# MCG-NJU/SparseBEV

Hardware: AMD Instinct MI355X
Metric: decoder samples/sec (6-cam T=8 900q r50_704x256, 6 layers, features resident in HBM) (higher is better)
Workload: dtype f32 (the two mixing GEMMs: f16x3 = fp32-class (default): fp32 operands as scaled fp16 hi + lo images, 3 products (hl, lh, hh), f32 accumulate on the 16-bit matrix core (csrc/gemm_bf16s.hip); max and rms error vs fp64 below the exact f32 MFMA kernels (tests/test_gpu_bf16s.py); mixing generator + out-; 1 GPU; c2: r50_704x256, 900 queries, T=8, bs=1 per GPU, 6 decoder layers, random-init weights, NCHW (reference layout, relayout inside the step: on demand -- only the feature units the sample points read) feature input; global_batch=1, parallelism=sample-sharded x1, launches_per_layer=6, query_order=False, shuffled_queries=False, relayout=on-demand

## Files before the change

### sparsebev_amd/csrc/gemm_bf16s.hip

```cpp
#include <atomic>
#include <cstdlib>
#include <type_traits>
#include "sbev_common.hpp"

#ifdef SBEV_EXP_NOSTORE
#define SBEV_EXP_STORE_COND && a.M < 0
#else
#define SBEV_EXP_STORE_COND
#endif
#ifdef SBEV_EXP_NOMFMA
#define SBEV_MFMA(A, B, C) ([&]() { asm volatile("" ::"v"(A), "v"(B)); return C; }())
#else
#define SBEV_MFMA(A, B, C) mfma16<PR::F16>(A, B, C)
#endif

#ifdef SBEV_EXP_TRACE
__device__ unsigned long long g_sbev_trace[2][512][8];
#define SBEV_TRACE(G_, SLOT_)                                                                               \
    if (blockIdx.x == 0 && (wave & 3) == 0 && lane == 0 && (G_) < 512) g_sbev_trace[wave >> 2][G_][SLOT_] = __builtin_readcyclecounter();
extern "C" int sbev_debug_trace_read(unsigned long long* out) {
    return (int)hipMemcpyFromSymbol(out, HIP_SYMBOL(g_sbev_trace), sizeof(g_sbev_trace));
}
#else
#define SBEV_TRACE(G_, SLOT_)
// ... 286 lines not shown
    typedef Fmt<MODE> PR;
    constexpr int NIMG = PR::NIMG;
    constexpr bool F16 = PR::F16;
    extern __shared__ __attribute__((aligned(16))) unsigned char lds[];
    constexpr Gen3Lds L{NIMG, RF};
    constexpr int AF = 2 * RF;
    constexpr int STAGE = L.stage();
    constexpr int NST = L.depth();
    constexpr bool EPI_LDS = L.patches();
    constexpr int EPI_LD = Gen3Lds::EPI_LD;
    constexpr int SLICES = L.slices_at();
    constexpr bool ISSUE_IN_COMPUTE = false;
    constexpr bool SPLIT_ACC = RF == 2;
    constexpr int NBLK = AF + 8;
    constexpr int NLMAX = (NBLK + 7) / 8;
    const int tid = threadIdx.x, lane = tid & 63;
    const int wave = __builtin_amdgcn_readfirstlane(tid >> 6);
    const int wr = wave >> 2, wc = wave & 3;
    SBEV_WGTIME(0, 0)
    const int M = a.M, nk = a.K / 16;
    const int lw = (int)xcd_contiguous(blockIdx.x, gridDim.x);
    const int rt = lw % a.ntm, ct0 = lw / a.ntm, cstep = (int)gridDim.x / a.ntm, nct = a.N / G_COLS;
    const int my_tiles = ct0 < nct ? (nct - ct0 + cstep - 1) / cstep : 0;
    const int G = my_tiles * nk;
    if (G == 0) return;
    const int f0 = a.rows.first(rt), nf = a.rows.count(rt);
    const int m0 = f0 * 32;
    int nfa = nf - RF * wr;
    nfa = nfa < 0 ? 0 : (nfa > RF ? RF : nfa);
    const int nlb = (NBLK - wave + 7) / 8;
    const int nl = nlb * NIMG;

    const unsigned voff = (unsigned)lane * 16u;
    const unsigned char* gbase[NLMAX];
    unsigned ldst[NLMAX];
    long long gstep[NLMAX];
    const int nfrag = (M + 31) / 32;
    const long long blkbytes = (long long)nk * NIMG * 1024;
#pragma unroll
    for (int j = 0; j < NLMAX; ++j) {
        const int q = wave + 8 * j;
        ldst[j] = (unsigned)(q * NIMG * 1024);
        if (q < AF) {
            int fb = f0 + q;
            fb = fb < nfrag ? fb : nfrag - 1;
            gbase[j] = reinterpret_cast<const unsigned char*>(a.Xs) + fb * blkbytes;
            gstep[j] = -(long long)nk * NIMG * 1024;
        } else {
            gbase[j] = reinterpret_cast<const unsigned char*>(a.Ws) + (long long)(ct0 * 8 + (q - AF)) * blkbytes;
            gstep[j] = (long long)(cstep * 8) * blkbytes - (long long)nk * NIMG * 1024;
        }
    }
    int lk = 0, lg = 0;
    auto issue_next = [&]() {
        if (lg >= G) return;
        const unsigned sb = (unsigned)((lg % NST) * STAGE);
#pragma unroll
        for (int j = 0; j < NLMAX; ++j) {
#ifndef SBEV_EXP_NOGLDS
            if (j < nlb) lds_dma<NIMG>(gbase[j], voff, sb + ldst[j]);
#endif
            gbase[j] += NIMG * 1024;
        }
        ++lg;
        if (++lk == nk) {
            lk = 0;
#pragma unroll
            for (int j = 0; j < NLMAX; ++j) gbase[j] += gstep[j];
        }
    };
    const int l31 = lane & 31, lh = lane >> 5;
    const unsigned aoff = (unsigned)(wr * RF) * (NIMG * 1024u) + voff;
    const unsigned boff = (unsigned)(AF + wc * 2) * (NIMG * 1024u) + voff;

    auto run = [&](auto nfa_c) {
        constexpr int NFA = decltype(nfa_c)::value;
        constexpr int NFR = NFA > 0 ? NFA : 1;
        bf16x8 xf[NFR][NIMG], wf[2][NIMG];
        constexpr int NFS = SPLIT_ACC ? NFR : 1;
        f32x16 acc[NFR][2], accs[NFS][2];
        auto init_acc = [&](int ti) {
#pragma unroll
            for (int fb = 0; fb < 2; ++fb) {
                const float bv = F16 ? 0.f : reinterpret_cast<const float*>(lds + SLICES)[ti * G_COLS + (wc * 2 + fb) * 32 + l31];
#pragma unroll
                for (int fa = 0; fa < NFR; ++fa)
#pragma unroll
                    for (int e = 0; e < 16; ++e) {
                        acc[fa][fb][e] = bv;
                        if constexpr (SPLIT_ACC) accs[fa][fb][e] = 0.f;
                    }
            }
        };
        auto store_tile = [&](int n0, int tix) {
            if constexpr (NFA > 0) {
                if constexpr (F16) {
                    const float* bs = reinterpret_cast<const float*>(lds + SLICES) + tix * G_COLS + wc * 64 + l31;
                    const float* cs = bs + my_tiles * G_COLS;
                    const float b0 = bs[0], b1 = bs[32], c0 = cs[0], c1 = cs[32];
#pragma unroll
                    for (int fa = 0; fa < NFA; ++fa)
#pragma unroll
                        for (int e = 0; e < 16; ++e) {
                            acc[fa][0][e] = fmaf(acc[fa][0][e], c0, b0);
                            acc[fa][1][e] = fmaf(acc[fa][1][e], c1, b1);
                        }
                }
                if (a.relu) {
#pragma unroll
                    for (int fa = 0; fa < NFA; ++fa)
#pragma unroll
                        for (int fb = 0; fb < 2; ++fb)
#pragma unroll
                            for (int e = 0; e < 16; ++e) acc[fa][fb][e] = fmaxf(acc[fa][fb][e], 0.f);
                }
                if constexpr (EPI_LDS) {
                    float* patch = reinterpret_cast<float*>(lds + NST * STAGE) + wave * (32 * EPI_LD);
                    const int pr = lane >> 3, pc = (lane & 7) * 4;
#pragma unroll
                    for (int fa = 0; fa < NFA; ++fa) {
                        const int r0 = m0 + (wr * RF + fa) * 32;
#pragma unroll
                        for (int fb = 0; fb < 2; ++fb) {
#pragma unroll
                            for (int e = 0; e < 16; ++e) patch[((e & 3) + 8 * (e >> 2) + 4 * lh) * EPI_LD + l31] = acc[fa][fb][e];
                            __builtin_amdgcn_wave_barrier();
                            f32x4 v[4];
#pragma unroll
                            for (int i = 0; i < 4; ++i) v[i] = *reinterpret_cast<const f32x4*>(patch + (pr + 8 * i) * EPI_LD + pc);
                            __builtin_amdgcn_wave_barrier();
                            float* y = a.Y + (long long)(r0 + pr) * a.ldy + n0 + wc * 64 + fb * 32 + pc;
#pragma unroll
                            for (int i = 0; i < 4; ++i)
                                if (r0 + pr + 8 * i < M SBEV_EXP_STORE_COND) *reinterpret_cast<f32x4*>(y + (long long)(8 * i) * a.ldy) = v[i];
                        }
                    }
                    return;
                }
#pragma unroll
                for (int fa = 0; fa < NFA; ++fa) {
                    const int r0 = m0 + (wr * RF + fa) * 32;
                    float* y = a.Y + (long long)(r0 + 4 * lh) * a.ldy + n0 + wc * 64 + l31;
                    if (r0 + 32 <= M SBEV_EXP_STORE_COND) {
#pragma unroll
                        for (int e = 0; e < 16; ++e) {
                            y[0] = acc[fa][0][e];
                            y[32] = acc[fa][1][e];
                            y += (e & 3) == 3 ? 5 * a.ldy : a.ldy;
                            asm volatile("" : "+v"(y));
                        }
                    } else {
#pragma unroll
                        for (int e = 0; e < 16; ++e) {
                            if (r0 + 4 * lh + (e & 3) + 8 * (e >> 2) < M SBEV_EXP_STORE_COND) {
                                y[0] = acc[fa][0][e];
                                y[32] = acc[fa][1][e];
                            }
                            y += (e & 3) == 3 ? 5 * a.ldy : a.ldy;
                            asm volatile("" : "+v"(y));
                        }
                    }
                }
            }
        };
        int cn0 = ct0 * G_COLS, ck = 0, ti = 0;
        bool pending = false;
        for (int i = tid; i < my_tiles * G_COLS; i += 512) {
            const int t = i / G_COLS, c = i - t * G_COLS;
            reinterpret_cast<float*>(lds + SLICES)[i] = a.bias ? a.bias[(ct0 + t * cstep) * G_COLS + c] : 0.f;
            if constexpr (F16)
                reinterpret_cast<float*>(lds + SLICES)[my_tiles * G_COLS + i] = a.colscale[(ct0 + t * cstep) * G_COLS + c] * a.xscale[1];
        }
        __syncthreads();
        init_acc(0);
#pragma unroll
        for (int i = 0; i < NST - 1; ++i) issue_next();
        wait_vmcnt_imm<0>();
        __syncthreads();
        if (wr == 1) phase_barrier();
        for (int g = 0; g < G; ++g) {
            SBEV_TRACE(g, 0)
            if constexpr (NFA > 0) {
                const unsigned char* st = lds + (g % NST) * STAGE;
#pragma unroll
                for (int img = 0; img < NIMG; ++img) {
                    wf[0][img] = *reinterpret_cast<const bf16x8*>(st + boff + img * 1024);
                    wf[1][img] = *reinterpret_cast<const bf16x8*>(st + boff + (NIMG + img) * 1024);
#pragma unroll
                    for (int fa = 0; fa < NFA; ++fa) xf[fa][img] = *reinterpret_cast<const bf16x8*>(st + aoff + (fa * NIMG + img) * 1024);
                }
            }
            SBEV_TRACE(g, 1)
            if constexpr (!ISSUE_IN_COMPUTE) issue_next();
            SBEV_TRACE(g, 2)
            {
                const int hi = lg - 1, need = g + 1 < G ? g + 1 : g;
                wait_vmcnt_n(hi > need ? (hi - need) * nl : 0);
            }
            if (pending) {
                store_tile(cn0, ti);
                cn0 += cstep * G_COLS;
                ++ti;
                init_acc(ti < my_tiles ? ti : 0);
                pending = false;
            }
            SBEV_TRACE(g, 3)
            phase_barrier();
            SBEV_TRACE(g, 4)
            if constexpr (ISSUE_IN_COMPUTE) issue_next();
            if constexpr (NFA > 0) {
#pragma unroll
                for (int p = 0; p < PR::N - 1; ++p)
#pragma unroll
                    for (int fa = 0; fa < NFA; ++fa)
#pragma unroll
                        for (int fb = 0; fb < 2; ++fb) {
                            if constexpr (SPLIT_ACC) accs[fa][fb] = SBEV_MFMA(xf[fa][PR::ia(p)], wf[fb][PR::ib(p)], accs[fa][fb]);
                            else acc[fa][fb] = SBEV_MFMA(xf[fa][PR::ia(p)], wf[fb][PR::ib(p)], acc[fa][fb]);
                        }
#pragma unroll
                for (int fa = 0; fa < NFA; ++fa)
#pragma unroll
                    for (int fb = 0; fb < 2; ++fb)
                        acc[fa][fb] = SBEV_MFMA(xf[fa][0], wf[fb][0], acc[fa][fb]);
            }
            if (++ck == nk) {
                ck = 0;
                pending = true;
                if constexpr (NFA > 0 && SPLIT_ACC) {
#pragma unroll
                    for (int fa = 0; fa < NFA; ++fa)
#pragma unroll
                        for (int fb = 0; fb < 2; ++fb) acc[fa][fb] += accs[fa][fb];
                }
            }
            SBEV_TRACE(g, 5)
            phase_barrier();
            SBEV_TRACE(g, 6)
        }
        if (wr == 0) phase_barrier();
        if (pending) store_tile(cn0, ti);
        SBEV_WGTIME(0, 1)
    };
    if (nfa == RF) run(std::integral_constant<int, RF>{});
    else if (nfa == RF - 1) run(std::integral_constant<int, RF - 1>{});
    else if (nfa == 0) run(std::integral_constant<int, 0>{});
    else if constexpr (RF == 4) {
        if (nfa == 2) run(std::integral_constant<int, 2>{});
        else run(std::integral_constant<int, 1>{});
    }
}

struct GenWsArgs {
    const unsigned short* Xs;
    const unsigned short* Ws;
    const float* bias;
    float* Y;
    int M, N;
    long long ldy;
    int relu;
    int nrs; RowSplit rows;
    int ntask;
    const float* colscale;
    const float* xscale;
    int lazy_on, lazy_esize;
    LazyArgs lazy;
    const uint32_t* skip_hdr;
};

#ifndef SBEV_WS_NCH
#define SBEV_WS_NCH 2
#endif
constexpr int WS_KS = 16;
constexpr int WS_FRAG = WS_KS * 2 * 1024;
constexpr int WS_SLOTS = 4;
constexpr int WS_LDS = WS_SLOTS * WS_FRAG;
static_assert(WS_LDS <= Gen3Lds::BUDGET, "the X ring fits the CU's LDS");

__device__ __forceinline__ void lds_barrier() {
    __builtin_amdgcn_sched_barrier(0);
    asm volatile("s_waitcnt lgkmcnt(0)\n\ts_barrier" ::: "memory");
    __builtin_amdgcn_sched_barrier(0);
}

template <int MODE, bool RELU>
__global__ __launch_bounds__(512) void gemm_f16s_gen_ws_kernel(const GenWsArgs a) {
    typedef Fmt<MODE> PR;
    static_assert(PR::NIMG == 2, "two-image modes only: the stationary weights are 128 registers");
    constexpr bool F16 = PR::F16;
    extern __shared__ __attribute__((aligned(16))) unsigned char lds[];
    if (a.skip_hdr && sbev::prefix_clean(a.skip_hdr)) return;
    const int lane = threadIdx.x & 63;
    const int wave = __builtin_amdgcn_readfirstlane((int)threadIdx.x >> 6);
    const int l31 = lane & 31, lh = lane >> 5;
    const unsigned voff = (unsigned)lane * 16u;
    const unsigned long long yb = (unsigned long long)a.Y;
    __amdgpu_buffer_rsrc_t yrs = __builtin_amdgcn_make_buffer_rsrc(
        reinterpret_cast<void*>(((unsigned long long)(unsigned)__builtin_amdgcn_readfirstlane((int)(unsigned)(yb >> 32)) << 32) |
                                (unsigned)__builtin_amdgcn_readfirstlane((int)(unsigned)yb)),
        0, (int)(unsigned)((long long)a.M * a.ldy * 4), 0x00020000);
    const unsigned ldyb = (unsigned)(a.ldy * 4);
    [[maybe_unused]] const int tid = (int)threadIdx.x;
    SBEV_WGTIME(1, 0)
    if (a.lazy_on) {
        float* wt = reinterpret_cast<float*>(lds);
        unsigned* list = reinterpret_cast<unsigned*>(lds + 8 * (LZ_TS * WLD * 4));
        unsigned* n_list = list + 4 * 512;
        if (a.lazy_esize == 4) lazy_scan_share<float>(a.lazy, blockIdx.x, gridDim.x, 512, wt, list, n_list);
        else lazy_scan_share<unsigned short>(a.lazy, blockIdx.x, gridDim.x, 512, wt, list, n_list);
        asm volatile("s_waitcnt vmcnt(0)" ::: "memory");
        __syncthreads();
    }

    {
        for (int task = (int)xcd_contiguous(blockIdx.x, gridDim.x); task < a.ntask; task += (int)gridDim.x) {
            const int ct = task / a.nrs, rs = task - ct * a.nrs;
            const int f0 = a.rows.first(rs), nf = a.rows.count(rs);
            if (nf <= 0) continue;
            const int n = ct * G_COLS + wave * 32 + l31;
            const float bv = a.bias ? a.bias[n] : 0.f;
            const float cv = F16 ? a.colscale[n] * a.xscale[1] : 1.f;
            const unsigned ycol = (unsigned)(4 * lh) * ldyb + (unsigned)n * 4u;
            const unsigned char* xg = reinterpret_cast<const unsigned char*>(a.Xs) + (long long)f0 * WS_FRAG + wave * 4096;
            auto issue = [&](int i) {
#ifndef SBEV_EXP_NOGLDS
                lds_dma<4>(xg + (long long)i * WS_FRAG, voff, (unsigned)((i % WS_SLOTS) * WS_FRAG + wave * 4096));
#endif
            };
            issue(0);
            if (nf > 1) issue(1);
            if (nf > 2) issue(2);
            __builtin_amdgcn_sched_barrier(0);
            bf16x8 wf[WS_KS][2];
            {
                const unsigned short* wb = a.Ws + ((long long)(ct * 8 + wave) * (WS_KS * 2) * 64 + lane) * 8;
#pragma unroll
                for (int ks = 0; ks < WS_KS; ++ks)
#pragma unroll
                    for (int img = 0; img < 2; ++img) wf[ks][img] = *reinterpret_cast<const bf16x8*>(wb + (ks * 2 + img) * 512);
            }
            __builtin_amdgcn_sched_barrier(0);
            wait_vmcnt_imm<32>();
            lds_barrier();
            f32x16 prev;
#pragma unroll
            for (int e = 0; e < 16; ++e) prev[e] = 0.f;
            for (int i = 0; i < nf; ++i) {
                SBEV_TRACE(i, 0)
                const unsigned char* st = lds + (i % WS_SLOTS) * WS_FRAG + voff;
                const unsigned yprev = i > 0 ? ycol + (unsigned)((f0 + i - 1) * 32) * ldyb : (ycol | 0x80000000u);
                constexpr int NCH = SBEV_WS_NCH;
                f32x16 accs[NCH];
#pragma unroll
                for (int c = 0; c < NCH; ++c)
#pragma unroll
                    for (int e = 0; e < 16; ++e) accs[c][e] = (F16 || c > 0) ? 0.f : bv;
                constexpr int NBLK = WS_KS / NCH;
                static_assert(WS_KS % NCH == 0 && NBLK % 2 == 0 && 16 % (NBLK / 2) == 0, "NCH divides the k-steps into an even number of blocks");
                constexpr int SPB = 16 / (NBLK / 2);
                bf16x8 xr[2][NCH][2];
#pragma unroll
                for (int c = 0; c < NCH; ++c) {
                    xr[0][c][0] = *reinterpret_cast<const bf16x8*>(st + (c * 2) * 1024);
                    xr[0][c][1] = *reinterpret_cast<const bf16x8*>(st + (c * 2 + 1) * 1024);
                }
#pragma unroll
                for (int blk = 0; blk < NBLK; ++blk) {
#ifndef SBEV_EXP_NOREAD
                    if (blk + 1 < NBLK) {
#pragma unroll
                        for (int c = 0; c < NCH; ++c) {
                            xr[(blk + 1) & 1][c][0] = *reinterpret_cast<const bf16x8*>(st + (((blk + 1) * NCH + c) * 2) * 1024);
                            xr[(blk + 1) & 1][c][1] = *reinterpret_cast<const bf16x8*>(st + (((blk + 1) * NCH + c) * 2 + 1) * 1024);
                        }
                    }
#endif
                    if (blk < NBLK / 2) {
#pragma unroll
                        for (int e = SPB * (blk % (NBLK / 2)); e < SPB * (blk % (NBLK / 2)) + SPB; ++e) {
                            const unsigned ro = (unsigned)((e & 3) + 8 * (e >> 2)) * ldyb;
#ifndef SBEV_EXP_NOSTORE
                            __builtin_amdgcn_raw_buffer_store_b32(__float_as_uint(prev[e]), yrs, (int)(yprev + ro), 0, 0);
#endif
                        }
                    }
#ifdef SBEV_EXP_NOREAD
                    const auto& xc = xr[0];
#else
                    const auto& xc = xr[blk & 1];
#endif
#pragma unroll
                    for (int p = 0; p < PR::N; ++p)
#pragma unroll
                        for (int c = 0; c < NCH; ++c) {
                            const int ks = blk * NCH + c;
                            if (p < PR::N - 1) accs[c] = SBEV_MFMA(xc[c][PR::ia(p)], wf[ks][PR::ib(p)], accs[c]);
                            else accs[c] = SBEV_MFMA(xc[c][0], wf[ks][0], accs[c]);
                        }
                    __builtin_amdgcn_sched_barrier(0);
                    if (blk == NBLK - 1) {
                        SBEV_TRACE(i, 1)
                        if (i + 2 < nf) wait_vmcnt_imm<4>();
                        else wait_vmcnt_imm<0>();
                        SBEV_TRACE(i, 2)
                        lds_barrier();
                        SBEV_TRACE(i, 3)
                        if (i + 3 < nf) issue(i + 3);
                        __builtin_amdgcn_sched_barrier(0);
                        SBEV_TRACE(i, 4)
                    }
                }
                f32x16 acc = accs[0];
#pragma unroll
                for (int c = 1; c < NCH; ++c) acc += accs[c];
#pragma unroll
                for (int e = 0; e < 16; ++e) {
                    const float v = F16 ? fmaf(acc[e], cv, bv) : acc[e];
                    prev[e] = RELU ? fmaxf(v, 0.f) : v;
                }
            }
            {
                const unsigned ylast = ycol + (unsigned)((f0 + nf - 1) * 32) * ldyb;
#pragma unroll
                for (int e = 0; e < 16; ++e)
                    __builtin_amdgcn_raw_buffer_store_b32(__float_as_uint(prev[e]), yrs, (int)(ylast + (unsigned)((e & 3) + 8 * (e >> 2)) * ldyb), 0, 0);
            }
        }
    }
    SBEV_WGTIME(1, 1)
}

struct OutArgs {
    const float* X;
    const unsigned short* Wp;
    float* P;
    int M, K;
    long long ldx;
    int nrt, S;
    float xup;
    const float* nscale;
    const float* xdev;
};

constexpr int O_IMG = 64 * 64;

template <int MODE>
__global__ __launch_bounds__(512) void gemm_bf16s_out3_kernel(const OutArgs a) {
    typedef Fmt<MODE> PR;
    constexpr int NIMG = PR::NIMG;
    extern __shared__ __attribute__((aligned(16))) unsigned char lds[];
    constexpr int HSTAGE = NIMG * O_IMG;
    constexpr int NST = 3;
    const int tid = threadIdx.x, lane = tid & 63;
    const int wave = __builtin_amdgcn_readfirstlane(tid >> 6);
    const int half = wave >> 2, wc = wave & 3;
    SBEV_WGTIME(2, 0)
    const unsigned logical = xcd_contiguous(blockIdx.x, gridDim.x);
    const int chunk = (int)(logical / (unsigned)a.nrt), rt = (int)(logical % (unsigned)a.nrt);
    const int M = a.M;
    const int m0 = rt * 64;
    const int nfa = (M - m0) > 32 ? 2 : 1;
    const int nslab = a.K / 32;
    const int c0 = (int)((long long)nslab * chunk / a.S), c1 = (int)((long long)nslab * (chunk + 1) / a.S);
    const int n_all = c1 - c0, n0h = (n_all + 1) / 2;
    const int sb = half == 0 ? c0 : c0 + n0h;
    const int nh = half == 0 ? n0h : n_all - n0h;

    const int th = tid & 255;
    const int srow = th >> 2, skq = th & 3;
    int grow = m0 + srow;
    grow = grow < M ? grow : M - 1;
    const float* xp = a.X + (long long)grow * a.ldx + skq * 8;
    const unsigned wofs = (unsigned)(srow * 64 + ((skq ^ ((srow >> 2) & 3)) * 16));
    unsigned char* hst = lds + half * (NST * HSTAGE);
    const int last_slab = nh > 0 ? sb + nh - 1 : c1 - 1;
    auto loadx = [&](int i, f32x4& v0, f32x4& v1) {
        int sl = sb + i;
        sl = sl < last_slab ? sl : last_slab;
#ifdef SBEV_EXP_HOTX
        sl = sl & 7;
#endif
        const float* p = xp + (long long)sl * 32;
        v0 = __builtin_nontemporal_load(reinterpret_cast<const f32x4*>(p));
        v1 = __builtin_nontemporal_load(reinterpret_cast<const f32x4*>(p + 4));
    };
    const float xup = a.xdev ? a.xdev[0] : a.xup;
    auto stagex = [&](int i, const f32x4 v0, const f32x4 v1) {
        u32x4 im[NIMG];
        split8m<MODE>(v0, v1, xup, im);
        unsigned char* st = hst + (i % NST) * HSTAGE + wofs;
#pragma unroll
        for (int img = 0; img < NIMG; ++img) *reinterpret_cast<u32x4*>(st + img * O_IMG) = im[img];
    };
    const int KS = a.K / 16;
    const unsigned short* wb0 = a.Wp + ((long long)(2 * wc) * KS * NIMG * 64 + lane) * 8;
    const unsigned short* wb1 = a.Wp + ((long long)(2 * wc + 1) * KS * NIMG * 64 + lane) * 8;
    auto loadw = [&](int i, int j, bf16x8 (&w)[2][NIMG]) {
        int sl = sb + i;
        sl = sl < last_slab ? sl : last_slab;
#ifdef SBEV_EXP_HOTW
        sl = sl & 7;
#endif
        const long long o = (long long)(2 * sl + j) * NIMG * 64 * 8;
#pragma unroll
        for (int img = 0; img < NIMG; ++img) {
            w[0][img] = *reinterpret_cast<const bf16x8*>(wb0 + o + img * 512);
            w[1][img] = *reinterpret_cast<const bf16x8*>(wb1 + o + img * 512);
        }
    };
    const int l31 = lane & 31, lh = lane >> 5;
    const unsigned swz = (unsigned)((lane >> 2) & 3);
    const unsigned fo0 = (unsigned)l31 * 64u + (((unsigned)lh) ^ swz) * 16u;
    const unsigned fo1 = (unsigned)l31 * 64u + ((2u + (unsigned)lh) ^ swz) * 16u;

    auto run = [&](auto nfa_c) {
        constexpr int NFA = decltype(nfa_c)::value;
        f32x16 acc[NFA][2];
#pragma unroll
        for (int fa = 0; fa < NFA; ++fa)
#pragma unroll
            for (int fb = 0; fb < 2; ++fb)
#pragma unroll
                for (int e = 0; e < 16; ++e) acc[fa][fb][e] = 0.f;
        f32x4 xa0, xa1, xb0, xb1;
        bf16x8 w[2][2][NIMG], xf[2][NFA][NIMG];
        loadx(0, xa0, xa1);
        loadx(1, xb0, xb1);
        loadw(0, 0, w[0]);
        loadw(0, 1, w[1]);
        stagex(0, xa0, xa1);
        loadx(2, xa0, xa1);
        stagex(1, xb0, xb1);
        loadx(3, xb0, xb1);
        __syncthreads();
        if (half == 1) phase_barrier();
#define SBEV_O3_SLAB(S_, X0, X1)                                                                            \
        {                                                                                                   \
                                                                                                 \
            {                                                                                               \
                SBEV_TRACE(S_, 0)                                                                           \
                const unsigned char* A = hst + ((S_) % NST) * HSTAGE;                                       \
                _Pragma("unroll") for (int img = 0; img < NIMG; ++img)                                      \
                    _Pragma("unroll") for (int fa = 0; fa < NFA; ++fa) {                                    \
                        xf[0][fa][img] = *reinterpret_cast<const bf16x8*>(A + fo0 + img * O_IMG + fa * 32 * 64); \
                        xf[1][fa][img] = *reinterpret_cast<const bf16x8*>(A + fo1 + img * O_IMG + fa * 32 * 64); \
                    }                                                                                       \
                if ((S_) >= nh) {       \
                    _Pragma("unroll") for (int j = 0; j < 2; ++j)                                           \
                        _Pragma("unroll") for (int fa = 0; fa < NFA; ++fa)                                  \
                            _Pragma("unroll") for (int img = 0; img < NIMG; ++img)                          \
                                _Pragma("unroll") for (int e = 0; e < 8; ++e) xf[j][fa][img][e] = (__bf16)0.f; \
                }                                                                                           \
                SBEV_TRACE(S_, 1)                                                                           \
                if ((S_) > 0) loadw((S_), 1, w[1]);           \
                SBEV_TRACE(S_, 2)                                                                           \
                SBEV_TRACE(S_, 3)                                                                           \
            }                                                                                               \
            phase_barrier();                                                                                \
            SBEV_TRACE(S_, 4)                                                                               \
             \
             \
             \
             \
            stagex((S_) + 2, X0, X1);                                                                       \
            loadx((S_) + 4, X0, X1);                                                                        \
            _Pragma("unroll") for (int p = 0; p < PR::N; ++p)                                               \
                _Pragma("unroll") for (int fa = 0; fa < NFA; ++fa)                                          \
                    _Pragma("unroll") for (int fb = 0; fb < 2; ++fb)                                        \
                        acc[fa][fb] = SBEV_MFMA(w[0][fb][PR::ib(p)], xf[0][fa][PR::ia(p)], acc[fa][fb]);    \
            _Pragma("unroll") for (int i = 0; i < PR::N * NFA * 2 - 2; ++i) {                               \
                __builtin_amdgcn_sched_group_barrier(0x008, 1, 0);                                          \
                __builtin_amdgcn_sched_group_barrier(0x002, 3, 0);                                          \
            }                                                                                               \
            __builtin_amdgcn_sched_group_barrier(0x008, 1, 0);                                              \
            __builtin_amdgcn_sched_group_barrier(0x200, NIMG, 0);                                           \
            __builtin_amdgcn_sched_group_barrier(0x008, 1, 0);                                              \
            __builtin_amdgcn_sched_group_barrier(0x020, 2, 0);                                              \
            __builtin_amdgcn_sched_barrier(0);                                                              \
            loadw((S_) + 1, 0, w[0]);                                                                       \
            _Pragma("unroll") for (int p = 0; p < PR::N; ++p)                                               \
                _Pragma("unroll") for (int fa = 0; fa < NFA; ++fa)                                          \
                    _Pragma("unroll") for (int fb = 0; fb < 2; ++fb)                                        \
                        acc[fa][fb] = SBEV_MFMA(w[1][fb][PR::ib(p)], xf[1][fa][PR::ia(p)], acc[fa][fb]);    \
            _Pragma("unroll") for (int i = 0; i < 2 * NIMG; ++i) {                                          \
                __builtin_amdgcn_sched_group_barrier(0x008, (PR::N * NFA * 2) / (2 * NIMG), 0);             \
                __builtin_amdgcn_sched_group_barrier(0x020, 1, 0);                                          \
            }                                                                                               \
            __builtin_amdgcn_sched_barrier(0);                                                              \
            SBEV_TRACE(S_, 5)                                                                               \
            phase_barrier();                                                                                \
            SBEV_TRACE(S_, 6)                                                                               \
        }
        int sl = 0;
        for (; sl + 1 < n0h; sl += 2) {
            SBEV_O3_SLAB(sl, xa0, xa1)
            SBEV_O3_SLAB(sl + 1, xb0, xb1)
        }
        if (sl < n0h) SBEV_O3_SLAB(sl, xa0, xa1)
#undef SBEV_O3_SLAB
        if (half == 0) phase_barrier();
        __syncthreads();
        f32x4* fold = reinterpret_cast<f32x4*>(lds) + (wc * 16) * 64 + lane;
        if (half == 1) {
#pragma unroll
            for (int fa = 0; fa < NFA; ++fa)
#pragma unroll
                for (int fb = 0; fb < 2; ++fb)
#pragma unroll
                    for (int g = 0; g < 4; ++g)
                        fold[((fa * 2 + fb) * 4 + g) * 64] = (f32x4){acc[fa][fb][4 * g], acc[fa][fb][4 * g + 1], acc[fa][fb][4 * g + 2], acc[fa][fb][4 * g + 3]};
        }
        __syncthreads();
        if (half == 1) return;
        float* out = a.P + (long long)chunk * M * 256 + wc * 64 + 4 * lh;
#pragma unroll
        for (int fa = 0; fa < NFA; ++fa) {
            const int row = m0 + fa * 32 + l31;
            if (row < M SBEV_EXP_STORE_COND) {
#pragma unroll
                for (int fb = 0; fb < 2; ++fb)
#pragma unroll
                    for (int g = 0; g < 4; ++g) {
                        const f32x4 o = fold[((fa * 2 + fb) * 4 + g) * 64];
                        f32x4 v = {acc[fa][fb][4 * g] + o[0], acc[fa][fb][4 * g + 1] + o[1], acc[fa][fb][4 * g + 2] + o[2], acc[fa][fb][4 * g + 3] + o[3]};
                        if constexpr (PR::F16) {
                            v *= *reinterpret_cast<const f32x4*>(a.nscale + wc * 64 + 4 * lh + fb * 32 + 8 * g);
                            if (a.xdev) v *= a.xdev[1];
                        }
                        *reinterpret_cast<f32x4*>(out + (long long)row * 256 + fb * 32 + 8 * g) = v;
                    }
            }
        }
        SBEV_WGTIME(2, 1)
    };
    if (nfa == 2) run(std::integral_constant<int, 2>{});
    else run(std::integral_constant<int, 1>{});
}

struct Out4Args {
    const unsigned* Xp;
    const unsigned short* Wp;
    float* P;
    int M, K;
    long long ldx;
    int ntm; RowSplit rows;
    int S;
    const float* nscale;
    unsigned* fold_sync;
    float* folded;
    int debug_drop;
};

constexpr int PAIR_NST = 3;
constexpr int PAIR_IMG = 128 * 32;
constexpr int PAIR_XSTAGE = 2 * PAIR_IMG;
constexpr int PAIR_WSLOT = 2 * 2 * 1024;
constexpr int PAIR_WRING0 = 2 * PAIR_NST * PAIR_XSTAGE;
constexpr int PAIR_FLD = 256 + 4;

__device__ __forceinline__ void pair_deinterleave(const u32x4 p, const u32x4 q, u32x4& hi, u32x4& lo) {
    hi = (u32x4){__builtin_amdgcn_perm(p.y, p.x, 0x05040100u), __builtin_amdgcn_perm(p.w, p.z, 0x05040100u),
                 __builtin_amdgcn_perm(q.y, q.x, 0x05040100u), __builtin_amdgcn_perm(q.w, q.z, 0x05040100u)};
    lo = (u32x4){__builtin_amdgcn_perm(p.y, p.x, 0x07060302u), __builtin_amdgcn_perm(p.w, p.z, 0x07060302u),
                 __builtin_amdgcn_perm(q.y, q.x, 0x07060302u), __builtin_amdgcn_perm(q.w, q.z, 0x07060302u)};
}

struct PairTile {
    int chunk, rt;
    int f0, nf;
    __device__ __forceinline__ explicit PairTile(const Out4Args& a) {
        const unsigned logical = xcd_contiguous(blockIdx.x, gridDim.x);
        const int c = (int)(logical / (unsigned)a.ntm), r = (int)(logical % (unsigned)a.ntm);
        chunk = c, rt = r;
        f0 = a.rows.first(r), nf = a.rows.count(r);
    }
    __device__ __forceinline__ int row0() const { return f0 * 32; }
    __device__ __forceinline__ static int kstep0(const Out4Args& a, int ch) { return (int)((long long)(a.K / 16) * ch / a.S); }
};

struct KSteps {
    int first, last;
    __device__ __forceinline__ int at(int i) const { return first + i < last ? first + i : last; }
};

template <bool HOOKS>
struct PairXRing {
    const unsigned* xp;
    unsigned wofs;
    unsigned char* ring;
    __device__ __forceinline__ PairXRing(const Out4Args& a, int tid, int row0, unsigned char* lds, int group) {
        const int th = tid & 255;
        const int srow = th >> 1, skq = th & 1;
        int grow = row0 + srow;
        grow = grow < a.M ? grow : a.M - 1;
        xp = a.Xp + (long long)grow * a.ldx + skq * 8;
        wofs = (unsigned)(srow * 32 + skq * 16);
        ring = lds + group * (PAIR_NST * PAIR_XSTAGE);
    }
    __device__ __forceinline__ unsigned char* slot(int i) const { return ring + (i % PAIR_NST) * PAIR_XSTAGE; }
    __device__ __forceinline__ void load(int sl, u32x4& v0, u32x4& v1) const {
#ifdef SBEV_EXP_HOTX
        if (HOOKS) sl = sl & 7;
#endif
        const unsigned* p = xp + (long long)sl * 16;
#ifdef SBEV_O4_XNT
        if (HOOKS) {
            v0 = __builtin_nontemporal_load(reinterpret_cast<const u32x4*>(p));
            v1 = __builtin_nontemporal_load(reinterpret_cast<const u32x4*>(p + 4));
            return;
        }
#endif
        v0 = *reinterpret_cast<const u32x4*>(p);
        v1 = *reinterpret_cast<const u32x4*>(p + 4);
    }
    __device__ __forceinline__ void stage(int i, const u32x4 p, const u32x4 q) const {
        unsigned char* st = slot(i) + wofs;
        pair_deinterleave(p, q, *reinterpret_cast<u32x4*>(st), *reinterpret_cast<u32x4*>(st + PAIR_IMG));
    }
};

struct FragLane {
    int l31, lh;
    unsigned fo;
    __device__ __forceinline__ explicit FragLane(int lane) : l31(lane & 31), lh(lane >> 5), fo((unsigned)l31 * 32u + (unsigned)lh * 16u) {}
};

template <int NFA>
__device__ __forceinline__ void read_x_frags(const unsigned char* stage, const FragLane fl, bf16x8 (&xf)[NFA][2]) {
    const unsigned char* A = stage + fl.fo;
#pragma unroll
    for (int img = 0; img < 2; ++img)
// ... 735 lines not shown
```

### sparsebev_amd/csrc/lazy_relayout.hpp

```cpp
#pragma once

constexpr int LZ_TS = 64;
struct LazyArgs {
    const void* const* table;
    int index[SBEV_MAX_LEVELS];
    const void* src[SBEV_MAX_LEVELS];
    void* out[SBEV_MAX_LEVELS];
    int S[SBEV_MAX_LEVELS];
    unsigned tiles[SBEV_MAX_LEVELS];
    unsigned base[SBEV_MAX_LEVELS + 1];
    int n_levels, R;
    unsigned* need;
    unsigned* done;
    int first, last;
};
inline void fill_lazy_args(LazyArgs& a, const sbev::LazyScan& z, bool first) {
    const sbev::LazyPlan& p = *z.plan;
    a.table = z.table; a.n_levels = p.n_levels; a.R = p.R; a.need = z.need; a.done = z.done; a.first = first; a.last = z.last;
    for (int l = 0; l < p.n_levels; ++l) {
        a.index[l] = z.table ? z.index[l] : 0;
        a.src[l] = z.table ? nullptr : z.src[l];
        a.out[l] = z.out[l];
        a.S[l] = p.S[l]; a.tiles[l] = p.tiles[l]; a.base[l] = p.base[l];
    }
    a.base[p.n_levels] = p.base[p.n_levels];
}

constexpr int LAZY_SCAN = 16;
__device__ __forceinline__ unsigned lazy_bytes_nonzero(unsigned w) {
    return ((w & 0xffu) ? 1u : 0u) | ((w & 0xff00u) ? 2u : 0u) | ((w & 0xff0000u) ? 4u : 0u) | ((w & 0xff000000u) ? 8u : 0u);
}
__device__ __forceinline__ unsigned lazy_bits_to_bytes(unsigned m) {
    return (m & 1u) | ((m & 2u) << 7) | ((m & 4u) << 14) | ((m & 8u) << 21);
}

__device__ __forceinline__ void lazy_locate(const LazyArgs& a, unsigned t, int& l, long long& img, int& ts) {
    l = 0;
#pragma unroll
    for (int j = 1; j < SBEV_MAX_LEVELS; ++j)
        if (j < a.n_levels && t >= a.base[j]) l = j;
    const unsigned rel = t - a.base[l];
    const unsigned i = rel / a.tiles[l];
    img = i;
    ts = (int)(rel - i * a.tiles[l]);
}

constexpr int WLD = 33;
__device__ __forceinline__ void lazy_wave_sync() {
    __builtin_amdgcn_fence(__ATOMIC_RELEASE, "wavefront");
    __builtin_amdgcn_wave_barrier();
    __builtin_amdgcn_fence(__ATOMIC_ACQUIRE, "wavefront");
}
__device__ __forceinline__ void lazy_move_unit_wave(const LazyArgs& a, int l, long long img, int ts, int g, float* wt, const float*) {
    const int lane = threadIdx.x & 63;
    const int R = a.R, S = a.S[l];
    const int s0 = ts * LZ_TS;
    const float* in = static_cast<const float*>(a.table ? a.table[a.index[l]] : a.src[l]) + img * R * S;
    float* out = static_cast<float*>(a.out[l]) + img * R * S;
    const int rg = g * LZ_TS;
    const bool vec = (S & 3) == 0;
    float4 v[2][8];
    if (vec) {
#pragma unroll
        for (int half = 0; half < 2; ++half)
#pragma unroll
            for (int i = 0; i < 8; ++i) {
                const int lr = 32 * half + (lane >> 4) + 4 * i, sx = s0 + (lane & 15) * 4;
                v[half][i] = make_float4(0.f, 0.f, 0.f, 0.f);
                if (sx < S) v[half][i] = *reinterpret_cast<const float4*>(in + (long long)(rg + lr) * S + sx);
            }
    }
#pragma unroll
    for (int half = 0; half < 2; ++half) {
        const int r0 = rg + 32 * half;
        if (vec) {
#pragma unroll
            for (int i = 0; i < 8; ++i) {
                const int lr = (lane >> 4) + 4 * i, ls = (lane & 15) * 4;
                wt[(ls + 0) * WLD + lr] = v[half][i].x;
                wt[(ls + 1) * WLD + lr] = v[half][i].y;
                wt[(ls + 2) * WLD + lr] = v[half][i].z;
                wt[(ls + 3) * WLD + lr] = v[half][i].w;
            }
        } else {
            for (int i = lane; i < 32 * LZ_TS; i += 64) {
                const int lr = i >> 6, ls = i & 63, sx = s0 + ls;
                wt[ls * WLD + lr] = sx < S ? in[(long long)(r0 + lr) * S + sx] : 0.f;
            }
        }
        lazy_wave_sync();
#pragma unroll
        for (int i = 0; i < 8; ++i) {
            const int ls = (lane >> 3) + 8 * i, lr = (lane & 7) * 4;
            const int sx = s0 + ls;
            if (sx < S) {
                const float4 o = make_float4(wt[ls * WLD + lr], wt[ls * WLD + lr + 1], wt[ls * WLD + lr + 2], wt[ls * WLD + lr + 3]);
                *reinterpret_cast<float4*>(out + (long long)sx * R + r0 + lr) = o;
            }
        }
        lazy_wave_sync();
    }
}
__device__ __forceinline__ void lazy_move_unit_wave(const LazyArgs& a, int l, long long img, int ts, int g, float* wtf, const unsigned short*) {
    unsigned* wt = reinterpret_cast<unsigned*>(wtf);
    const int lane = threadIdx.x & 63;
    const int R = a.R, S = a.S[l];
    const int r0 = g * 64, s0 = ts * 64;
    const unsigned short* in = static_cast<const unsigned short*>(a.table ? a.table[a.index[l]] : a.src[l]) + img * R * S;
    unsigned short* out = static_cast<unsigned short*>(a.out[l]) + img * R * S;
    if ((S & 3) == 0) {
        uint2 lo[8], hi[8];
#pragma unroll
        for (int i = 0; i < 8; ++i) {
            const int cp = (lane >> 4) + 4 * i, sx = s0 + 4 * (lane & 15);
            lo[i] = make_uint2(0u, 0u); hi[i] = make_uint2(0u, 0u);
            if (sx < S) {
                lo[i] = *reinterpret_cast<const uint2*>(in + (long long)(r0 + 2 * cp) * S + sx);
                hi[i] = *reinterpret_cast<const uint2*>(in + (long long)(r0 + 2 * cp + 1) * S + sx);
            }
        }
#pragma unroll
        for (int i = 0; i < 8; ++i) {
            const int cp = (lane >> 4) + 4 * i, q = lane & 15;
            wt[(4 * q + 0) * WLD + cp] = __builtin_amdgcn_perm(hi[i].x, lo[i].x, 0x05040100u);
            wt[(4 * q + 1) * WLD + cp] = __builtin_amdgcn_perm(hi[i].x, lo[i].x, 0x07060302u);
            wt[(4 * q + 2) * WLD + cp] = __builtin_amdgcn_perm(hi[i].y, lo[i].y, 0x05040100u);
            wt[(4 * q + 3) * WLD + cp] = __builtin_amdgcn_perm(hi[i].y, lo[i].y, 0x07060302u);
        }
    } else {
        for (int i = lane; i < 32 * 64; i += 64) {
            const int cp = i >> 6, ls = i & 63, sx = s0 + ls;
            unsigned w = 0u;
            if (sx < S) w = (unsigned)in[(long long)(r0 + 2 * cp) * S + sx] | ((unsigned)in[(long long)(r0 + 2 * cp + 1) * S + sx] << 16);
            wt[ls * WLD + cp] = w;
        }
    }
    lazy_wave_sync();
#pragma unroll
    for (int i = 0; i < 8; ++i) {
        const int px = (lane >> 3) + 8 * i, k = lane & 7;
        const int sx = s0 + px;
        if (sx < S) {
            const unsigned* t = &wt[px * WLD + 4 * k];
            *reinterpret_cast<uint4*>(out + (long long)sx * R + r0 + 8 * k) = make_uint4(t[0], t[1], t[2], t[3]);
        }
    }
    lazy_wave_sync();
}


template <typename ET>
__device__ __forceinline__ void lazy_scan_share(const LazyArgs& a, unsigned wg, unsigned nwg, int per_batch, float* wtiles, unsigned* list,
                                                unsigned* n_list) {
    const int tid = threadIdx.x;
    const int wave = tid >> 6, nwave = (int)blockDim.x >> 6;
    const unsigned total = a.base[a.n_levels];
    const unsigned per_wg = (total + nwg - 1) / nwg;
    for (unsigned b0 = 0; b0 < per_wg; b0 += (unsigned)per_batch) {
        if (tid == 0) *n_list = 0u;
        __syncthreads();
        const unsigned slot = b0 + (unsigned)tid;
        const unsigned t = slot * nwg + wg;
        if (tid < per_batch && slot < per_wg && t < total) {
            const unsigned nw = a.need[t], dw = a.done[t];
            if (nw != 0u) {
                const unsigned pend = lazy_bytes_nonzero(nw) & ~lazy_bytes_nonzero(dw);
                if (pend) {
                    a.done[t] = dw | lazy_bits_to_bytes(pend);
                    const unsigned at = atomicAdd(n_list, (unsigned)__builtin_popcount(pend));
                    unsigned k = 0;
                    for (int g = 0; g < 4; ++g)
                        if ((pend >> g) & 1u) list[at + k++] = (unsigned)tid | ((unsigned)g << 16);
                }
                if (a.last) a.need[t] = 0u;
            }
        }
        __syncthreads();
        const unsigned n = *n_list;
        for (unsigned i = (unsigned)wave; i < n; i += (unsigned)nwave) {
            const unsigned e = list[i];
            int l, ts;
            long long img;
            lazy_locate(a, (b0 + (e & 0xffffu)) * nwg + wg, l, img, ts);
            lazy_move_unit_wave(a, l, img, ts, (int)(e >> 16), wtiles + wave * (LZ_TS * WLD), static_cast<const ET*>(nullptr));
        }
        __syncthreads();
    }
}
```

Baseline: 571.2 samples/s.

## Overlap stationary weight loads with lazy relayout scan in generator GEMM

When lazy relayout is active, the generator weight-stationary GEMM now issues its first task's register-resident weight loads before the lazy scan/move pass, so the global-memory latency hides under the relayout work. The first scan batch is restructured: need/done words and level source pointers are loaded up front, and barriers use an lgkmcnt-only wait so the outstanding weight loads are not drained. Tile location uses a precomputed per-level pointer array instead of re-reading the table. The cost is higher register pressure while the scan runs (128 weight registers held live) and more code complexity, plus a full vmcnt(0) wait before the first task.

```diff
diff --git a/sparsebev_amd/csrc/gemm_bf16s.hip b/sparsebev_amd/csrc/gemm_bf16s.hip
--- a/sparsebev_amd/csrc/gemm_bf16s.hip
+++ b/sparsebev_amd/csrc/gemm_bf16s.hip
@@ -612,20 +612,35 @@
     const unsigned ldyb = (unsigned)(a.ldy * 4);
     [[maybe_unused]] const int tid = (int)threadIdx.x;
     SBEV_WGTIME(1, 0)
-    if (a.lazy_on) {
-        float* wt = reinterpret_cast<float*>(lds);
-        unsigned* list = reinterpret_cast<unsigned*>(lds + 8 * (LZ_TS * WLD * 4));
-        unsigned* n_list = list + 4 * 512;
-        if (a.lazy_esize == 4) lazy_scan_share<float>(a.lazy, blockIdx.x, gridDim.x, 512, wt, list, n_list);
-        else lazy_scan_share<unsigned short>(a.lazy, blockIdx.x, gridDim.x, 512, wt, list, n_list);
-        asm volatile("s_waitcnt vmcnt(0)" ::: "memory");
-        __syncthreads();
-    }
-
-    {
-        for (int task = (int)xcd_contiguous(blockIdx.x, gridDim.x); task < a.ntask; task += (int)gridDim.x) {
+
+    auto run = [&](auto lazy_c) {
+        constexpr bool LAZY = decltype(lazy_c)::value;
+        bf16x8 wf[WS_KS][2];
+        auto load_w = [&](int ct) {
+            const unsigned short* wb = a.Ws + ((long long)(ct * 8 + wave) * (WS_KS * 2) * 64 + lane) * 8;
+#pragma unroll
+            for (int ks = 0; ks < WS_KS; ++ks)
+#pragma unroll
+                for (int img = 0; img < 2; ++img) wf[ks][img] = *reinterpret_cast<const bf16x8*>(wb + (ks * 2 + img) * 512);
+        };
+        int task = (int)xcd_contiguous(blockIdx.x, gridDim.x);
+        [[maybe_unused]] bool w_under_scan = false;
+        if constexpr (LAZY) {
+            float* wt = reinterpret_cast<float*>(lds);
+            unsigned* list = reinterpret_cast<unsigned*>(lds + 8 * (LZ_TS * WLD * 4));
+            unsigned* n_list = list + 4 * 512;
+            w_under_scan = task < a.ntask;
+            auto request = [&] { load_w(w_under_scan ? task / a.nrs : 0); };
+            if (a.lazy_esize == 4) lazy_scan_share_under<float>(a.lazy, blockIdx.x, gridDim.x, 512, wt, list, n_list, 8, request);
+            else lazy_scan_share_under<unsigned short>(a.lazy, blockIdx.x, gridDim.x, 512, wt, list, n_list, 8, request);
+            asm volatile("s_waitcnt vmcnt(0)" ::: "memory");
+            __syncthreads();
+        }
+        for (; task < a.ntask; task += (int)gridDim.x) {
             const int ct = task / a.nrs, rs = task - ct * a.nrs;
             const int f0 = a.rows.first(rs), nf = a.rows.count(rs);
+            const bool have_w = LAZY && w_under_scan;
+            if constexpr (LAZY) w_under_scan = false;
             if (nf <= 0) continue;
             const int n = ct * G_COLS + wave * 32 + l31;
             const float bv = a.bias ? a.bias[n] : 0.f;
@@ -641,16 +656,10 @@
             if (nf > 1) issue(1);
             if (nf > 2) issue(2);
             __builtin_amdgcn_sched_barrier(0);
-            bf16x8 wf[WS_KS][2];
-            {
-                const unsigned short* wb = a.Ws + ((long long)(ct * 8 + wave) * (WS_KS * 2) * 64 + lane) * 8;
-#pragma unroll
-                for (int ks = 0; ks < WS_KS; ++ks)
-#pragma unroll
-                    for (int img = 0; img < 2; ++img) wf[ks][img] = *reinterpret_cast<const bf16x8*>(wb + (ks * 2 + img) * 512);
-            }
+            if (!have_w) load_w(ct);
             __builtin_amdgcn_sched_barrier(0);
-            wait_vmcnt_imm<32>();
+            if (have_w) wait_vmcnt_imm<0>();
+            else wait_vmcnt_imm<32>();
             lds_barrier();
             f32x16 prev;
 #pragma unroll
@@ -736,7 +745,9 @@
                     __builtin_amdgcn_raw_buffer_store_b32(__float_as_uint(prev[e]), yrs, (int)(ylast + (unsigned)((e & 3) + 8 * (e >> 2)) * ldyb), 0, 0);
             }
         }
-    }
+    };
+    if (a.lazy_on) run(std::true_type{});
+    else run(std::false_type{});
     SBEV_WGTIME(1, 1)
 }
 
diff --git a/sparsebev_amd/csrc/lazy_relayout.hpp b/sparsebev_amd/csrc/lazy_relayout.hpp
--- a/sparsebev_amd/csrc/lazy_relayout.hpp
+++ b/sparsebev_amd/csrc/lazy_relayout.hpp
@@ -46,17 +46,25 @@
 }
 
 constexpr int WLD = 33;
+struct LazyLevel {
+    const void* in;
+    void* out;
+    int S;
+};
+__device__ __forceinline__ LazyLevel lazy_level(const LazyArgs& a, int l) {
+    return {a.table ? a.table[a.index[l]] : a.src[l], a.out[l], a.S[l]};
+}
 __device__ __forceinline__ void lazy_wave_sync() {
     __builtin_amdgcn_fence(__ATOMIC_RELEASE, "wavefront");
     __builtin_amdgcn_wave_barrier();
     __builtin_amdgcn_fence(__ATOMIC_ACQUIRE, "wavefront");
 }
-__device__ __forceinline__ void lazy_move_unit_wave(const LazyArgs& a, int l, long long img, int ts, int g, float* wt, const float*) {
+__device__ __forceinline__ void lazy_move_unit_wave(const LazyLevel lv, int R, long long img, int ts, int g, float* wt, const float*) {
     const int lane = threadIdx.x & 63;
-    const int R = a.R, S = a.S[l];
+    const int S = lv.S;
     const int s0 = ts * LZ_TS;
-    const float* in = static_cast<const float*>(a.table ? a.table[a.index[l]] : a.src[l]) + img * R * S;
-    float* out = static_cast<float*>(a.out[l]) + img * R * S;
+    const float* in = static_cast<const float*>(lv.in) + img * R * S;
+    float* out = static_cast<float*>(lv.out) + img * R * S;
     const int rg = g * LZ_TS;
     const bool vec = (S & 3) == 0;
     float4 v[2][8];
@@ -101,13 +109,13 @@
         lazy_wave_sync();
     }
 }
-__device__ __forceinline__ void lazy_move_unit_wave(const LazyArgs& a, int l, long long img, int ts, int g, float* wtf, const unsigned short*) {
+__device__ __forceinline__ void lazy_move_unit_wave(const LazyLevel lv, int R, long long img, int ts, int g, float* wtf, const unsigned short*) {
     unsigned* wt = reinterpret_cast<unsigned*>(wtf);
     const int lane = threadIdx.x & 63;
-    const int R = a.R, S = a.S[l];
+    const int S = lv.S;
     const int r0 = g * 64, s0 = ts * 64;
-    const unsigned short* in = static_cast<const unsigned short*>(a.table ? a.table[a.index[l]] : a.src[l]) + img * R * S;
-    unsigned short* out = static_cast<unsigned short*>(a.out[l]) + img * R * S;
+    const unsigned short* in = static_cast<const unsigned short*>(lv.in) + img * R * S;
+    unsigned short* out = static_cast<unsigned short*>(lv.out) + img * R * S;
     if ((S & 3) == 0) {
         uint2 lo[8], hi[8];
 #pragma unroll
@@ -149,41 +157,100 @@
 }
 
 
+__device__ __forceinline__ void lazy_scan_mark(const LazyArgs& a, unsigned t, unsigned nw, unsigned dw, unsigned* list, unsigned* n_list) {
+    if (nw != 0u) {
+        const unsigned pend = lazy_bytes_nonzero(nw) & ~lazy_bytes_nonzero(dw);
+        if (pend) {
+            a.done[t] = dw | lazy_bits_to_bytes(pend);
+            const unsigned at = atomicAdd(n_list, (unsigned)__builtin_popcount(pend));
+            unsigned k = 0;
+            for (int g = 0; g < 4; ++g)
+                if ((pend >> g) & 1u) list[at + k++] = (unsigned)threadIdx.x | ((unsigned)g << 16);
+        }
+        if (a.last) a.need[t] = 0u;
+    }
+}
+template <typename ET, typename Locate>
+__device__ __forceinline__ void lazy_scan_move(const LazyArgs& a, unsigned b0, unsigned wg, unsigned nwg, float* wtiles, const unsigned* list,
+                                               unsigned n, int nwave, Locate&& locate) {
+    const int wave = (int)threadIdx.x >> 6;
+    for (unsigned i = (unsigned)wave; i < n; i += (unsigned)nwave) {
+        const unsigned e = list[i];
+        LazyLevel lv;
+        int ts;
+        long long img;
+        locate((b0 + (e & 0xffffu)) * nwg + wg, lv, img, ts);
+        lazy_move_unit_wave(lv, a.R, img, ts, (int)(e >> 16), wtiles + wave * (LZ_TS * WLD), static_cast<const ET*>(nullptr));
+    }
+}
+
 template <typename ET>
 __device__ __forceinline__ void lazy_scan_share(const LazyArgs& a, unsigned wg, unsigned nwg, int per_batch, float* wtiles, unsigned* list,
-                                                unsigned* n_list) {
+                                                unsigned* n_list, unsigned b_from = 0u) {
     const int tid = threadIdx.x;
-    const int wave = tid >> 6, nwave = (int)blockDim.x >> 6;
     const unsigned total = a.base[a.n_levels];
     const unsigned per_wg = (total + nwg - 1) / nwg;
-    for (unsigned b0 = 0; b0 < per_wg; b0 += (unsigned)per_batch) {
+    for (unsigned b0 = b_from; b0 < per_wg; b0 += (unsigned)per_batch) {
         if (tid == 0) *n_list = 0u;
         __syncthreads();
         const unsigned slot = b0 + (unsigned)tid;
         const unsigned t = slot * nwg + wg;
         if (tid < per_batch && slot < per_wg && t < total) {
             const unsigned nw = a.need[t], dw = a.done[t];
-            if (nw != 0u) {
-                const unsigned pend = lazy_bytes_nonzero(nw) & ~lazy_bytes_nonzero(dw);
-                if (pend) {
-                    a.done[t] = dw | lazy_bits_to_bytes(pend);
-                    const unsigned at = atomicAdd(n_list, (unsigned)__builtin_popcount(pend));
-                    unsigned k = 0;
-                    for (int g = 0; g < 4; ++g)
-                        if ((pend >> g) & 1u) list[at + k++] = (unsigned)tid | ((unsigned)g << 16);
-                }
-                if (a.last) a.need[t] = 0u;
-            }
-        }
-        __syncthreads();
-        const unsigned n = *n_list;
-        for (unsigned i = (unsigned)wave; i < n; i += (unsigned)nwave) {
-            const unsigned e = list[i];
-            int l, ts;
-            long long img;
-            lazy_locate(a, (b0 + (e & 0xffffu)) * nwg + wg, l, img, ts);
-            lazy_move_unit_wave(a, l, img, ts, (int)(e >> 16), wtiles + wave * (LZ_TS * WLD), static_cast<const ET*>(nullptr));
-        }
-        __syncthreads();
-    }
-}
+            lazy_scan_mark(a, t, nw, dw, list, n_list);
+        }
+        __syncthreads();
+        lazy_scan_move<ET>(a, b0, wg, nwg, wtiles, list, *n_list, (int)blockDim.x >> 6, [&](unsigned tile, LazyLevel& lv, long long& img, int& ts) {
+            int l;
+            lazy_locate(a, tile, l, img, ts);
+            lv = lazy_level(a, l);
+        });
+        __syncthreads();
+    }
+}
+
+__device__ __forceinline__ void lazy_lds_barrier() {
+    __builtin_amdgcn_sched_barrier(0);
+    asm volatile("s_waitcnt lgkmcnt(0)\n\ts_barrier" ::: "memory");
+    __builtin_amdgcn_sched_barrier(0);
+}
+
+template <typename ET, typename Request>
+__device__ __forceinline__ void lazy_scan_share_under(const LazyArgs& a, unsigned wg, unsigned nwg, int per_batch, float* wtiles,
+                                                      unsigned* list, unsigned* n_list, int nwave, Request&& request) {
+    const int tid = threadIdx.x;
+    const unsigned total = a.base[a.n_levels];
+    const unsigned per_wg = (total + nwg - 1) / nwg;
+    const unsigned t = (unsigned)tid * nwg + wg;
+    const bool mine = tid < per_batch && (unsigned)tid < per_wg && t < total;
+    unsigned nw = 0u, dw = 0u;
+    if (mine) { nw = a.need[t]; dw = a.done[t]; }
+    const void* in[SBEV_MAX_LEVELS];
+#pragma unroll
+    for (int j = 0; j < SBEV_MAX_LEVELS; ++j) in[j] = j < a.n_levels ? (a.table ? a.table[a.index[j]] : a.src[j]) : nullptr;
+    __builtin_amdgcn_sched_barrier(0);
+    request();
+    __builtin_amdgcn_sched_barrier(0);
+    if (tid == 0) *n_list = 0u;
+    lazy_lds_barrier();
+    if (mine) lazy_scan_mark(a, t, nw, dw, list, n_list);
+    lazy_lds_barrier();
+    lazy_scan_move<ET>(a, 0u, wg, nwg, wtiles, list, *n_list, nwave, [&](unsigned tile, LazyLevel& lv, long long& img, int& ts) {
+        lv = LazyLevel{in[0], a.out[0], a.S[0]};
+        unsigned base = a.base[0], tiles = a.tiles[0];
+#pragma unroll
+        for (int j = 1; j < SBEV_MAX_LEVELS; ++j)
+            if (j < a.n_levels && tile >= a.base[j]) {
+                lv = LazyLevel{in[j], a.out[j], a.S[j]};
+                base = a.base[j];
+                tiles = a.tiles[j];
+            }
+        const unsigned rel = tile - base, i = rel / tiles;
+        img = i;
+        ts = (int)(rel - i * tiles);
+    });
+    if ((unsigned)per_batch < per_wg) {
+        __syncthreads();
+        lazy_scan_share<ET>(a, wg, nwg, per_batch, wtiles, list, n_list, (unsigned)per_batch);
+    }
+}
```

Measured after the change: 578.3 samples/s (median of 6 runs). 1.2% higher.
